# zhixuan-lin/IODINE

Measured on AMD Instinct MI355X. Metric: refinement_iters_per_s, higher is better.
Workload: dtype f32 tensors; conv products from 3 f16 MFMAs on hi+lo splits: >= 22 bits relative to the 8x16-cell maximum (tile-relative), f32 accumulate; 1 GPU; CLEVR6 128x128, K=7, T=5, batch 32/GPU, train step (forward + backward + fused Adam step, noise drawn inside the step); step=train, global_batch=32, slots=7, iters=5, img_size=128, hip_graph=False

## Files before the change

iodine_amd/csrc/iodine_testops.cpp:

```cpp
#include "iodine_internal.h"

namespace {

class OpScratch {
    char* base_ = nullptr;
    std::vector<size_t> off_;
public:
    OpScratch(const char* who, std::initializer_list<size_t> region_bytes)
    {
        size_t total = 0;
        for (size_t b : region_bytes) { off_.push_back(total); total += (b + 15) & ~(size_t)15; }
        const hipError_t e = hipMalloc((void**)&base_, std::max<size_t>(total, 16));
        if (e != hipSuccess) { base_ = nullptr; free_fail(IODINE_ERR_HIP, std::string(who) + ": hipMalloc of " + std::to_string(total) + " bytes of scratch: " + hipGetErrorString(e)); }
    }
    ~OpScratch() { if (base_) (void)hipFree(base_); }
    OpScratch(const OpScratch&) = delete;
    OpScratch& operator=(const OpScratch&) = delete;
    bool ok() const { return base_ != nullptr; }
    template <typename T = float> T* at(int region) const { return reinterpret_cast<T*>(base_ + off_[region]); }
    Pack pack(int region) const { return Pack{at<char>(region), at(region + 1)}; }
};

int op_done(const char* who, hipStream_t st, hipError_t e) { return free_hip(who, e == hipSuccess ? hipStreamSynchronize(st) : e); }

constexpr size_t META_BYTES = 64;

}

extern "C" {

int iodine_op_conv3x3(void* stream, int mode, const float* in, const float* w, const float* bias, const float* aux,
                      float* out, int n, int ih, int iw, int w_o, int w_i, int cin_pad, int cout, int stride, int epi,
                      int tflip)
{
    hipStream_t st = (hipStream_t)stream;
    const bool square_cc = cin_pad == cout && w_o == cout && w_i == cout && ih == iw;
    switch (mode) {
    case IODINE_CONV_S2_FWD: case IODINE_CONV_S2_DGRAD: case IODINE_CONV_S2_FWD_F32: case IODINE_CONV_S2_DGRAD_F32: {
        const bool fwd = mode == IODINE_CONV_S2_FWD || mode == IODINE_CONV_S2_FWD_F32;
        const int f32 = mode == IODINE_CONV_S2_FWD_F32 || mode == IODINE_CONV_S2_DGRAD_F32;
        const int cp = fwd ? (cin_pad == 20 ? 32 : (cin_pad == 12 || cin_pad == 8 ? 16 : cin_pad)) : cin_pad;
        OpScratch scr("iodine_op_conv3x3(s2 f16x3)", {wpk_s2_tile_bytes(cp, cout), META_BYTES});
        if (!scr.ok()) return IODINE_ERR_HIP;
        const Pack p = scr.pack(0);
        hipError_t e = f32 ? launch_pack_conv_weights_s2f32(st, w, w_o, w_i, cp, cout, fwd ? 0 : 2, p.data)
                           : launch_pack_conv_weights_f16(st, w, w_o, w_i, cp, cout, fwd ? 0 : 2, p.meta, p.data);
        if (e == hipSuccess)
            e = fwd ? launch_conv3x3_s2_f16x3(st, in, p.data, p.meta, bias, out, n, ih, cin_pad, cout, nullptr, 0, f32)
                    : launch_conv3x3_s2_dgrad_f16x3(st, in, p.data, p.meta, aux, out, n, ih, cout, f32);
        return op_done("iodine_op_conv3x3(s2 f16x3)", st, e);
    }
    case IODINE_CONV_WS: case IODINE_CONV_WS_B: case IODINE_CONV_WS_1P: {
        if (!square_cc || ih % 16 != 0) return free_fail(IODINE_ERR_INVALID, "iodine_op_conv3x3(ws): shape");
        const size_t tf = conv_ws_tmax_floats(n, ih);
        OpScratch scr("iodine_op_conv3x3(ws)", {wpk_ws_bytes(cout), META_BYTES, tf * sizeof(float), tf * sizeof(float)});
        if (!scr.ok()) return IODINE_ERR_HIP;
        const Pack p = scr.pack(0);
        float *tin = scr.at(2), *tout = scr.at(3);
        hipError_t e = launch_pack_conv_weights_ws(st, w, cout, tflip, p.meta, p.data);
        if (e == hipSuccess) e = launch_cell_max(st, in, tin, n, ih, cout);
        if (e == hipSuccess) e = launch_conv3x3_ws_f16x3(st, in, p.data, p.meta, bias, aux, out, tin, tout, n, ih, cout, epi, 0, mode == IODINE_CONV_WS_1P ? 1 : 3);
        return op_done("iodine_op_conv3x3(ws)", st, e);
    }
    case IODINE_CONV_S2WS: case IODINE_CONV_S2WS_F32: {
        if (!square_cc || !conv3x3_s2ws_ok(ih, cout)) return free_fail(IODINE_ERR_INVALID, "iodine_op_conv3x3(s2ws): shape");
        const bool f32 = mode == IODINE_CONV_S2WS_F32;
        OpScratch scr("iodine_op_conv3x3(s2ws)", {wpk_ws_bytes(cout), META_BYTES});
        if (!scr.ok()) return IODINE_ERR_HIP;
        const Pack p = scr.pack(0);
        hipError_t e = f32 ? launch_pack_conv_weights_ws32(st, w, cout, 0, p.data) : launch_pack_conv_weights_ws(st, w, cout, 0, p.meta, p.data);
        if (e == hipSuccess) e = launch_conv3x3_s2ws_f16x3(st, in, p.data, p.meta, bias, out, n, ih, cout, f32);
        return op_done("iodine_op_conv3x3(s2ws)", st, e);
    }
    case IODINE_CONV_WS_F32: {
        if (!square_cc || ih % 16 != 0) return free_fail(IODINE_ERR_INVALID, "iodine_op_conv3x3(ws f32): shape");
        OpScratch scr("iodine_op_conv3x3(ws f32)", {wpk_ws_bytes(cout)});
        if (!scr.ok()) return IODINE_ERR_HIP;
        hipError_t e = launch_pack_conv_weights_ws32(st, w, cout, tflip, scr.at<char>(0));
        if (e == hipSuccess) e = launch_conv3x3_ws_f32(st, in, scr.at<char>(0), bias, aux, out, n, ih, cout, epi, 0);
        return op_done("iodine_op_conv3x3(ws f32)", st, e);
    }
#ifdef IODINE_WITH_WINO
    case IODINE_CONV_WINO: {
        if (!square_cc || ih % 16 != 0) return free_fail(IODINE_ERR_INVALID, "iodine_op_conv3x3(wino): shape");
        const size_t tf = conv_ws_tmax_floats(n, ih);
        OpScratch scr("iodine_op_conv3x3(wino)", {conv_wino_wpk_bytes(cout), META_BYTES, tf * sizeof(float), tf * sizeof(float), conv_wino_scratch_floats(cout) * sizeof(float)});
        if (!scr.ok()) return IODINE_ERR_HIP;
        const Pack p = scr.pack(0);
        float *tin = scr.at(2), *tout = scr.at(3);
        hipError_t e = launch_pack_conv_weights_wino(st, w, cout, tflip, p.meta, p.data, scr.at(4));
        if (e == hipSuccess) e = launch_cell_max(st, in, tin, n, ih, cout);
        if (e == hipSuccess) e = launch_conv3x3_wino_f16x3(st, in, p.data, p.meta, bias, aux, out, tin, tout, n, ih, cout, epi, 0);
        return op_done("iodine_op_conv3x3(wino)", st, e);
    }
#endif
    case IODINE_CONV_TILE_F16: {
        OpScratch scr("iodine_op_conv3x3(f16x3)", {wpk_tile_f16_bytes(cin_pad, cout), META_BYTES});
        if (!scr.ok()) return IODINE_ERR_HIP;
        const Pack p = scr.pack(0);
        hipError_t e = launch_pack_conv_weights_f16(st, w, w_o, w_i, cin_pad, cout, tflip, p.meta, p.data);
        if (e == hipSuccess) e = launch_conv3x3_tile_f16x3(st, in, p.data, p.meta, bias, aux, out, n, ih, cin_pad, cout, epi, 0);
        return op_done("iodine_op_conv3x3(f16x3)", st, e);
    }
    default: break;
    }
    OpScratch scr("iodine_op_conv3x3", {wpk_tile_f32_bytes(cin_pad, cout)});
    if (!scr.ok()) return IODINE_ERR_HIP;
    float* wpk = scr.at(0);
    hipError_t e = launch_pack_conv_weights(st, w, w_o, w_i, cin_pad, cout, tflip, wpk);
    if (e == hipSuccess && mode == IODINE_CONV_TILE_F32)
        e = (ih == iw && stride == 1) ? launch_conv3x3_tile(st, in, wpk, bias, aux, out, n, ih, cin_pad, cout, epi) : hipErrorInvalidValue;
    else if (e == hipSuccess)
        e = launch_conv3x3_gather(st, in, wpk, bias, out, n, ih, iw, cin_pad, cout, stride);
    return op_done("iodine_op_conv3x3", st, e);
}

int iodine_op_dec_out(void* stream, const float* in, const float* w, const float* bias, float* out, int n, int s, int c)
{
    hipStream_t st = (hipStream_t)stream;
    OpScratch scr("iodine_op_dec_out", {wpk_out_taps_bytes(c)});
    if (!scr.ok()) return IODINE_ERR_HIP;
    hipError_t e = launch_pack_dec_out(st, w, scr.at(0), c);
    if (e == hipSuccess) e = launch_dec_out(st, in, scr.at(0), bias, out, n, s, c);
    return op_done("iodine_op_dec_out", st, e);
}

int iodine_op_dec_out_f16x3(void* stream, const float* in, const float* w, const float* bias, float* out, int n, int s, int c, int variant)
{
    hipStream_t st = (hipStream_t)stream;
    if (s % 16 != 0 || (c != 64 && c != 32)) return free_fail(IODINE_ERR_INVALID, "iodine_op_dec_out_f16x3: shape");
    OpScratch scr("iodine_op_dec_out_f16x3", {std::max(wpk_out_gemm_bytes(c), wpk_out_rows32_bytes(c)), META_BYTES, conv_ws_tmax_floats(n, s) * sizeof(float)});
    if (!scr.ok()) return IODINE_ERR_HIP;
    const Pack p = scr.pack(0);
    float* tin = scr.at(2);
    hipError_t e = launch_pack_dec_out_gemm(st, w, c, p.meta, p.data);
    if (e == hipSuccess) e = launch_cell_max(st, in, tin, n, s, c);
    if (e == hipSuccess && variant == IODINE_DEC_OUT_ROWS_F32) {
        e = launch_pack_dec_out_rows32(st, w, c, (float*)p.data);
        if (e == hipSuccess) e = launch_dec_out_rows_f16x3(st, in, p.data, nullptr, bias, out, n, s, c, nullptr, 1);
    } else if (e == hipSuccess)
        e = variant == IODINE_DEC_OUT_ROWS ? launch_dec_out_rows_f16x3(st, in, p.data, p.meta, bias, out, n, s, c, tin)
                                           : launch_dec_out_stream_f16x3(st, in, p.data, p.meta, bias, out, n, s, c, variant == IODINE_DEC_OUT_TILES_NOMAX ? nullptr : tin);
    return op_done("iodine_op_dec_out_f16x3", st, e);
}

int iodine_op_conv3x3_wgrad(void* stream, const float* in, const float* d, float* gw, float* gb, int n, int s, int ci_pad,
                            int ci_real, int co, int stride)
{
    hipStream_t st = (hipStream_t)stream;
    const int cmax = std::max(std::max(ci_pad, co), 32);
    OpScratch scr("iodine_op_conv3x3_wgrad", {sizeof(float) * 512 * 4 * 9 * cmax * cmax, sizeof(float) * WGRAD_FOLD * 9 * cmax * cmax, sizeof(float) * 512 * 64});
    if (!scr.ok()) return IODINE_ERR_HIP;
    float *part = scr.at(0), *fold = scr.at(1), *part_b = scr.at(2);
    int nparts = 0, cip = 0, nb = 0;
    hipError_t e;
    if (stride == 1 && co == 4) {
        e = launch_dec_out_wgrad_gemm_f16x3(st, in, d, part, part_b, n, s, ci_pad, &nparts, &nb);
        if (e == hipSuccess) e = launch_wgrad_reduce(st, part, nparts, ci_pad, 4, 4, ci_real, ci_real, 1.f, gw, fold);
    } else if (stride == 1) {
        e = launch_conv3x3_wgrad_f16x3_ws(st, in, d, part, part_b, n, s, ci_pad, co, &nparts, &cip, &nb);
        if (e == hipSuccess) e = launch_wgrad_reduce(st, part, nparts, ci_pad, cip, co, ci_real, ci_real, 1.f, gw, fold);
    } else {
        e = launch_conv3x3_s2_wgrad_f16x3(st, in, d, part, part_b, n, s, ci_pad, co, &nparts, &cip, &nb, nullptr, 0, stride == IODINE_WGRAD_STRIDE2_F32);
        if (e == hipSuccess) e = launch_wgrad_reduce(st, part, nparts, cip, co, co, ci_real, ci_real, 1.f, gw, fold);
    }
    if (e == hipSuccess) e = launch_colsum(st, part_b, nb, co, co, 1.f, gb);
    return op_done("iodine_op_conv3x3_wgrad", st, e);
}

int iodine_op_gen_conv(void* stream, int mode, const float* in, const float* w, const float* bias, const float* aux, float* out, float* gb,
                       int n, int si, int ci, int ldc, int co, int k, int s, int elu)
{
    hipStream_t st = (hipStream_t)stream;
    if (mode < IODINE_GEN_FWD || mode > IODINE_GEN_WGRAD || s < 1 || s > 8 || (k != 3 && k != 5 && k != 7) || ldc < ci) return free_fail(IODINE_ERR_INVALID, "iodine_op_gen_conv: argument");
    const unsigned chmask = (elu & 0x100) ? ((unsigned)elu >> 9) : 0xffffffffu;
    elu &= 1;
    OpScratch scr("iodine_op_gen_conv", {wpk_gen_bytes(k, ldc, co), mode == IODINE_GEN_WGRAD ? gen_wgrad_scratch_floats(ci, co, k) * sizeof(float) : 0});
    if (!scr.ok()) return IODINE_ERR_HIP;
    float* wt = scr.at(0);
    hipError_t e = hipSuccess;
    if (mode == IODINE_GEN_FWD) {
        e = launch_gen_pack_weights(st, w, co, ci, k, wt);
        if (e == hipSuccess) e = launch_gen_conv_fwd(st, in, wt, bias, out, n, si, ci, ldc, co, k, s, elu, chmask);
    } else if (mode == IODINE_GEN_DGRAD) {
        e = launch_gen_pack_weights(st, w, co, ldc, k, wt);
        if (e == hipSuccess) e = launch_gen_conv_dgrad(st, in, wt, aux, out, n, si, ci, ldc, co, k, s);
    } else {
        e = launch_gen_conv_wgrad(st, in, aux, scr.at(1), n, si, ci, ldc, ci, co, k, s, 1.f, out, gb, chmask);
    }
    return op_done("iodine_op_gen_conv", st, e);
}

int iodine_op_gen_conv_tier(int mode, int si, int ci, int ldc, int co, int k, int s)
{
    if (mode < IODINE_GEN_FWD || mode > IODINE_GEN_WGRAD || si < 1 || ci < 1 || co < 1 || s < 1 || s > 8 || (k != 3 && k != 5 && k != 7) || ldc < ci) return -1;
    const GenTierSel sel = gen_conv_tier(mode, si, ci, ldc, co, k, s);
    return (int)sel.tier | (sel.np << 8) | (sel.seg << 16);
}

int iodine_op_gen_l0(void* stream, int mode, const float* z, const float* w, const float* bias, const float* dpre, float* out, float* gw,
                     float* gb, float* dz, int n, int L, int s, int co, int k, int ld, float alpha)
{
    hipStream_t st = (hipStream_t)stream;
    if (mode < IODINE_GEN_FWD || mode > IODINE_GEN_DGRAD || n < 1 || L < 1 || s < 1 || co < 1 || k < 1 || k > GEN_L0_KMAX || k % 2 == 0 || !z || !w
        || (mode == IODINE_GEN_FWD && (!bias || !out)) || (mode == IODINE_GEN_DGRAD && (!dpre || !dz || ld < L || (alpha != 0.f && (!gw || !gb)))))
        return free_fail(IODINE_ERR_INVALID, "iodine_op_gen_l0: argument");
    OpScratch scr("iodine_op_gen_l0", {wpk_gen_bytes(k, L + 2, co), (size_t)s * sizeof(float), mode == IODINE_GEN_FWD ? (size_t)s * s * co * sizeof(float) : 0,
                                       gen_l0_scratch_floats(n, s, co, k) * sizeof(float)});
    if (!scr.ok()) return IODINE_ERR_HIP;
    float *wt = scr.at(0), *lin = scr.at(1), *cterm = scr.at(2), *tmp = scr.at(3);
    std::vector<float> hlin((size_t)s);
    iodine_linspace_host(s, hlin.data());
    hipError_t e = hipMemcpyAsync(lin, hlin.data(), (size_t)s * sizeof(float), hipMemcpyHostToDevice, st);
    if (e == hipSuccess) e = hipStreamSynchronize(st);
// ... 230 lines not shown
```

iodine_amd/csrc/kernels_convws.hip:

```cpp
#include "common.h"
#include "pack_bodies.h"
#include <cstdio>
#include <vector>

__global__ void pack_conv_weights_ws_kernel(const float* __restrict__ src, int C, int tflip, const float* __restrict__ meta,
                                            _Float16* __restrict__ dst)
{
    const float scale = meta[0];
    const size_t total = pack_ws_total(C);
    for (size_t idx = (size_t)blockIdx.x * blockDim.x + threadIdx.x; idx < total; idx += (size_t)gridDim.x * blockDim.x)
        dst[idx] = pack_ws_element(src, C, tflip, scale, idx);
}

__global__ __launch_bounds__(1024) void weight_scale_ws_kernel(const float* __restrict__ w, int n, float* __restrict__ meta)
{
    __shared__ float s_red[16];
    weight_scale_block(w, n, meta, s_red);
}

hipError_t launch_pack_conv_weights_ws(hipStream_t st, const float* src, int C, int tflip, float* meta, void* dst)
{
    hipLaunchKernelGGL(weight_scale_ws_kernel, dim3(1), dim3(1024), 0, st, src, C * C * 9, meta);
    const size_t total = wpk_ws_vecs(C) * 8;
    hipLaunchKernelGGL(pack_conv_weights_ws_kernel, dim3((unsigned)((total + 255) / 256)), dim3(256), 0, st, src, C, tflip,
                       meta, (_Float16*)dst);
    return hipGetLastError();
}

__global__ __launch_bounds__(256) void cell_max_kernel(const float* __restrict__ x, float* __restrict__ tmax, int S, int C)
{
    const int cells_x = S / 16, cells_y = S / 8;
    const int cell = blockIdx.x;
    const int cx = cell % cells_x, cy = (cell / cells_x) % cells_y, n = cell / (cells_x * cells_y);
    const float4* base = reinterpret_cast<const float4*>(x + (size_t)n * S * S * C);
    const int c4 = C / 4;
    float m = 0.f;
    for (int i = threadIdx.x; i < 128 * c4; i += 256) {
        const int px = i / c4, q = i % c4;
        const float4 v = base[((size_t)(cy * 8 + px / 16) * S + cx * 16 + px % 16) * c4 + q];
        m = fmaxf(m, fmaxf(fmaxf(fabsf(v.x), fabsf(v.y)), fmaxf(fabsf(v.z), fabsf(v.w))));
    }
    __shared__ float s_red[4];
    m = wave_max_f32(m);
    if ((threadIdx.x & 63) == 0) s_red[threadIdx.x >> 6] = m;
    __syncthreads();
    if (threadIdx.x < 4) tmax[(size_t)cell * 4 + threadIdx.x] = fmaxf(fmaxf(s_red[0], s_red[1]), fmaxf(s_red[2], s_red[3]));
}

hipError_t launch_cell_max(hipStream_t st, const float* x, float* tmax, int N, int S, int C)
{
    hipLaunchKernelGGL(cell_max_kernel, dim3(N * (S / 16) * (S / 8)), dim3(256), 0, st, x, tmax, S, C);
    return hipGetLastError();
}

#ifdef IODINE_TILE_PROF
__device__ unsigned g_ws_prof[TP_MAXBLK * 8];
__device__ unsigned long long g_ws_ts[TP_MAXBLK * 16];
__device__ unsigned long long g_ws_se[TP_MAXBLK * 2];
static void ws_prof_dump(hipStream_t st, int blocks, int ntiles);
#endif

template <int SEGS>
IOD_DEVINL float pixel_lane_sum(float v)
{
    {
        const auto r = __builtin_amdgcn_permlane32_swap(__float_as_uint(v), __float_as_uint(v), false, false);
        v = __uint_as_float(r[0]) + __uint_as_float(r[1]);
    }
    {
        const auto r = __builtin_amdgcn_permlane16_swap(__float_as_uint(v), __float_as_uint(v), false, false);
        v = __uint_as_float(r[0]) + __uint_as_float(r[1]);
    }
    if constexpr (SEGS == 8) v += __uint_as_float(__builtin_amdgcn_update_dpp(0u, __float_as_uint(v), 0x128, 0xf, 0xf, false));
    return v;
}

constexpr int ws_pxb(int c) { return 160; }
constexpr int ws_bpc(int c, int epi) { return 2; }

template <int C, int EPI, bool F32 = false, int NPROD = 3>
__global__ __launch_bounds__(256, ws_bpc(C, EPI))
void conv3x3_ws_f16x3_kernel(const float* __restrict__ in, const uint4* __restrict__ wpk, const float* __restrict__ wmeta,
                             const float* __restrict__ bias, const float* __restrict__ aux, float* __restrict__ out,
                             const float* __restrict__ tmax_in, float* __restrict__ tmax_out, int S, int lgS, int ntiles, int rev)
{
    constexpr int NCG = C / 16;
    constexpr int NPG = 4 / NCG;
    constexpr int RW = 8 / NPG;
    constexpr int NCHUNK = C / 32;
    constexpr int HC = 18, HR = 10, NPX = HC * HR;
    constexpr int PXB = ws_pxb(C);
    constexpr int EPS = C * 4 + 32;
    constexpr int BUFB = ((NPX + 1) * PXB > 128 * EPS ? (NPX + 1) * PXB : 128 * EPS);
    constexpr int NIN = (NPX * 8 + 255) / 256;
    constexpr int NS = (RW + 2) * 3;
    constexpr bool XPOSE = true;
    constexpr bool ROWS = EPI == EPI_L0ROWS || EPI == EPI_L0ROWSX;
    constexpr int NQ = EPI == EPI_L0ROWSX ? 4 : 3;
    constexpr bool GRADF = EPI == EPI_MUL_ELUGRAD || ROWS;
    constexpr int SEGS = C / 4, PPI = 64 / SEGS, NEP = 32 / PPI;
    static_assert(C == 64 || C == 32, "channel counts of the shipped decoders");
    static_assert(EPI == EPI_BIAS_ELU || EPI == EPI_MUL_ELUGRAD || ROWS, "epilogue");
    static_assert(NPROD == 3 || (NPROD == 1 && !F32), "products per term: the split (3) or hi.hi alone (1, fp16 form only)");
    constexpr bool ONE = NPROD == 1;

    extern __shared__ __attribute__((aligned(16))) unsigned char smem_b[];

    using std::integral_constant;
    const int tid = threadIdx.x, lane = tid & 63;
    const int wv = __builtin_amdgcn_readfirstlane(tid >> 6);
    const int cg = wv % NCG, pg = wv / NCG;
    const int lpx = lane & 15, lkb = lane >> 4;

#define WS_BLOAD4(dst, voff, rsrc, soff) \
    asm volatile("buffer_load_dwordx4 %0, %1, %2, %3 offen" : "=v"(dst) : "v"(voff), "s"(rsrc), "s"(soff) : "memory")
#ifndef WS_STORE_POLICY
#define WS_STORE_POLICY 0
#endif
#if WS_STORE_POLICY == 1
#define WS_STORE_MOD " nt"
#elif WS_STORE_POLICY == 2
#define WS_STORE_MOD " sc1"
#elif WS_STORE_POLICY == 3
#define WS_STORE_MOD " sc0 sc1"
#else
#define WS_STORE_MOD ""
#endif
#define WS_BSTORE4(src, voff, rsrc, soff) \
    asm volatile("s_nop 4\n\tbuffer_store_dwordx4 %0, %1, %2, %3 offen" WS_STORE_MOD "\n\ts_nop 1" :: "v"(src), "v"(voff), "s"(rsrc), "s"(soff) : "memory")
#define WS_SGPR_SETTLE(rsrc, soff) asm volatile("s_nop 4" :: "s"(rsrc), "s"(soff) : "memory")

    using wreg_t = std::conditional_t<F32, f32x4, f16x8>;
    wreg_t wh[NCHUNK][9], wl[NCHUNK][9];
    auto load_weights = [&]() {
        const uint4* wp = wpk + (size_t)cg * NCHUNK * 9 * 2 * 64 + lane;
#pragma unroll
        for (int c = 0; c < NCHUNK; ++c)
#pragma unroll
            for (int t = 0; t < 9; ++t) {
                if constexpr (ONE) {
                    const uint4 h = wp[((c * 9 + t) * 2 + 0) * 64];
                    __builtin_memcpy(&wh[c][t], &h, 16);
                } else {
                const uint4 h = wp[((c * 9 + t) * 2 + 0) * 64], l = wp[((c * 9 + t) * 2 + 1) * 64];
                __builtin_memcpy(&wh[c][t], &h, 16);
                __builtin_memcpy(&wl[c][t], &l, 16);
                }
            }
#pragma unroll
        for (int c = 0; c < NCHUNK; ++c)
#pragma unroll
            for (int t = 0; t < 9; ++t) {
                if constexpr (ONE) asm volatile("" : "+v"(wh[c][t]));
                else asm volatile("" : "+v"(wh[c][t]), "+v"(wl[c][t]));
            }
    };
    float inv_w = 1.f;
    if constexpr (!F32) inv_w = wmeta[1];
    const float xstep_u = __uint_as_float(__builtin_amdgcn_readfirstlane(__float_as_uint(__fdiv_rn(2.f, (float)(S - 1)))));
    (void)xstep_u;

    const unsigned lds_base = (unsigned)(size_t)(__attribute__((address_space(3))) unsigned char*)smem_b;
    const unsigned lw0 = (unsigned)((tid >> 3) * PXB + (tid & 7) * (F32 ? 16 : 8));
    const bool last_idle = tid + (NIN - 1) * 256 >= NPX * 8;
    const unsigned fr_base = lds_base + (unsigned)(((pg * RW) * HC + lpx) * PXB + lkb * 16);

    const int tiles_x = S >> 4, tiles_y = S >> 3, lg_tx = lgS - 4, lg_tpi = 2 * lgS - 7;
    const int nblk = gridDim.x;
    const int xcd = blockIdx.x & 7, bix = blockIdx.x >> 3, bpx = (nblk + 7) >> 3;
    const int per_xcd = (ntiles + 7) >> 3;
    const int t_begin = xcd * per_xcd, t_end = min(ntiles, t_begin + per_xcd);

    f32x4 rin[NIN];
    auto tile_coords = [&](int t, int& n, int& ty, int& tx) {
        const int tt = rev ? ntiles - 1 - t : t;
        n = tt >> lg_tpi;
        ty = (tt >> lg_tx) & (tiles_y - 1); tx = tt & (tiles_x - 1);
    };
    float tmv = 0.f;
    auto issue_tmax = [&](int t) {
        int n, ty, tx;
        tile_coords(t, n, ty, tx);
        const int cell = min(lane >> 2, 8);
        const int cy = min(max(ty + cell / 3 - 1, 0), tiles_y - 1), cx = min(max(tx + cell % 3 - 1, 0), tiles_x - 1);
        const float* p = tmax_in + ((((size_t)n << lg_tpi) + (cy << lg_tx) + cx) << 2) + (lane & 3);
        asm volatile("global_load_dword %0, %1, off" : "=v"(tmv) : "v"(p) : "memory");
    };
    auto issue_loads = [&](int t, int chunk) {
        int n, ty, tx;
        tile_coords(t, n, ty, tx);
        const i32x4 rsrc = iod_make_rsrc(in + (size_t)n * S * S * C, (unsigned)(S * S * C * 4));
        unsigned goff[NIN];
#pragma unroll
        for (int k = 0; k < NIN; ++k) {
            const int px = (tid >> 3) + 32 * k;
            const int hy = (px * 3641) >> 16, hx = px - hy * HC;
            const int gy = ty * 8 - 1 + hy, gx = tx * 16 - 1 + hx;
            const bool ok = (k < NIN - 1 || px < NPX) && (unsigned)gy < (unsigned)S && (unsigned)gx < (unsigned)S;
            goff[k] = ok ? (unsigned)(((((gy << lgS) + gx) * C) << 2) + ((tid & 7) << 4)) : 0x80000000u;
        }
        const int soff = chunk * 128;
        WS_SGPR_SETTLE(rsrc, soff);
#pragma unroll
        for (int k = 0; k < NIN; ++k) WS_BLOAD4(rin[k], goff[k], rsrc, soff);
    };
    const int t0 = t_begin + bix;
    const int nstage = t0 < t_end ? ((t_end - t0 + bpx - 1) / bpx) * NCHUNK : 0;
    auto issue_stage = [&](int s) {
        const int t = t0 + (s / NCHUNK) * bpx, c = s % NCHUNK;
        issue_loads(t, c);
        if constexpr (!F32) { if (c == 0) issue_tmax(t); }
    };
    auto vm_wait = [&](auto nc) {
        constexpr int nleft = decltype(nc)::value;
        asm volatile("s_waitcnt vmcnt(%0)" :: "n"(nleft) : "memory");
#pragma unroll
        for (int k = 0; k < NIN; ++k) asm volatile("" : "+v"(rin[k]));
        asm volatile("" : "+v"(tmv));
        __builtin_amdgcn_sched_barrier(0);
    };

    f32x4 acc[RW];

    auto convert_k = [&](auto kc, int buf, float scale) {
        constexpr int k = decltype(kc)::value;
        unsigned char* sb = smem_b + buf * BUFB;
        f32x4 v = rin[k];
        if constexpr (F32) {
            const unsigned o32 = (k == NIN - 1 && last_idle) ? (unsigned)(NPX * PXB) : lw0 + (unsigned)(k * 32 * PXB);
            *reinterpret_cast<f32x4*>(sb + o32) = v;
        } else if constexpr (ONE) {
            v.x *= scale; v.y *= scale; v.z *= scale; v.w *= scale;
            typedef _Float16 hr2 __attribute__((ext_vector_type(2)));
            const hr2 h01 = {(_Float16)v.x, (_Float16)v.y}, h23 = {(_Float16)v.z, (_Float16)v.w};
            uint2 hi;
            __builtin_memcpy(&hi.x, &h01, 4); __builtin_memcpy(&hi.y, &h23, 4);
            const unsigned o = (k == NIN - 1 && last_idle) ? (unsigned)(NPX * PXB) : lw0 + (unsigned)(k * 32 * PXB);
            *reinterpret_cast<uint2*>(sb + o) = hi;
        } else {
        v.x *= scale; v.y *= scale; v.z *= scale; v.w *= scale;
        typedef __fp16 h2 __attribute__((ext_vector_type(2)));
        const h2 h01 = __builtin_amdgcn_cvt_pkrtz(v.x, v.y), h23 = __builtin_amdgcn_cvt_pkrtz(v.z, v.w);
        const h2 l01 = __builtin_amdgcn_cvt_pkrtz(v.x - (float)h01.x, v.y - (float)h01.y), l23 = __builtin_amdgcn_cvt_pkrtz(v.z - (float)h23.x, v.w - (float)h23.y);
        uint2 hi, lo;
        __builtin_memcpy(&hi.x, &h01, 4); __builtin_memcpy(&hi.y, &h23, 4);
        __builtin_memcpy(&lo.x, &l01, 4); __builtin_memcpy(&lo.y, &l23, 4);
        const unsigned o = (k == NIN - 1 && last_idle) ? (unsigned)(NPX * PXB) : lw0 + (unsigned)(k * 32 * PXB);
        *reinterpret_cast<uint2*>(sb + o) = hi;
        *reinterpret_cast<uint2*>(sb + o + 64) = lo;
        }
    };

    constexpr int NST = ROWS ? 2 * NQ : NEP + (F32 ? 0 : 1);

#define WS_DSR128(dst, addr, off) asm volatile("ds_read_b128 %0, %1 offset:%2" : "=v"(dst) : "v"(addr), "n"(off))
    struct Frag { wreg_t h, l; };
    constexpr int HOOK0 = 3;
    auto compute = [&](auto cc, int buf, bool has_next, bool next_after_epi, float next_scale_same, float& next_scale, bool has_next2,
                       int next2_stage) {
        constexpr int c = decltype(cc)::value;
        const unsigned base = fr_base + (unsigned)(buf * BUFB);
        Frag f[2];
        auto LOADF = [](auto sc, Frag& fr, unsigned b) {
            constexpr int s = decltype(sc)::value;
            constexpr int hr = s / 3, dx = s % 3;
            constexpr int off = (hr * HC + dx) * PXB;
            WS_DSR128(fr.h, b, off);
            if constexpr (!ONE) WS_DSR128(fr.l, b, off + 64);
        };
        auto MMA = [&](auto sc, const Frag& fr) {
            constexpr int s = decltype(sc)::value;
            constexpr int hr = s / 3, dx = s % 3;
            if constexpr (F32) {
#pragma unroll
                for (int j = 0; j < 4; ++j)
#pragma unroll
                    for (int dy = 0; dy < 3; ++dy) {
                        const int y = hr - dy;
                        if (y >= 0 && y < RW) acc[y] = __builtin_amdgcn_mfma_f32_16x16x4f32(wh[c][dy * 3 + dx][j], fr.h[j], acc[y], 0, 0, 0);
                    }
#pragma unroll
                for (int j = 0; j < 4; ++j)
#pragma unroll
                    for (int dy = 0; dy < 3; ++dy) {
                        const int y = hr - dy;
                        if (y >= 0 && y < RW) acc[y] = __builtin_amdgcn_mfma_f32_16x16x4f32(wl[c][dy * 3 + dx][j], fr.l[j], acc[y], 0, 0, 0);
                    }
            } else if constexpr (ONE) {
#pragma unroll
                for (int dy = 0; dy < 3; ++dy) {
                    const int y = hr - dy;
                    if (y >= 0 && y < RW) acc[y] = __builtin_amdgcn_mfma_f32_16x16x32_f16(wh[c][dy * 3 + dx], fr.h, acc[y], 0, 0, 0);
                }
            } else {
#pragma unroll
            for (int dy = 0; dy < 3; ++dy) {
                const int y = hr - dy;
                if (y >= 0 && y < RW) acc[y] = __builtin_amdgcn_mfma_f32_16x16x32_f16(wh[c][dy * 3 + dx], fr.l, acc[y], 0, 0, 0);
            }
#pragma unroll
            for (int dy = 0; dy < 3; ++dy) {
                const int y = hr - dy;
                if (y >= 0 && y < RW) acc[y] = __builtin_amdgcn_mfma_f32_16x16x32_f16(wl[c][dy * 3 + dx], fr.h, acc[y], 0, 0, 0);
            }
#pragma unroll
            for (int dy = 0; dy < 3; ++dy) {
                const int y = hr - dy;
                if (y >= 0 && y < RW) acc[y] = __builtin_amdgcn_mfma_f32_16x16x32_f16(wh[c][dy * 3 + dx], fr.h, acc[y], 0, 0, 0);
            }
            }
        };
        LOADF(integral_constant<int, 0>{}, f[0], base);
        auto step = [&](auto sc) {
            constexpr int s = decltype(sc)::value;
            if constexpr (s + 1 < NS) {
                LOADF(integral_constant<int, (s + 1 < NS ? s + 1 : 0)>{}, f[(s + 1) & 1], base);
                if constexpr (ONE) asm volatile("s_waitcnt lgkmcnt(1)" ::: "memory");
                else asm volatile("s_waitcnt lgkmcnt(2)" ::: "memory");
            } else {
                asm volatile("s_waitcnt lgkmcnt(0)" ::: "memory");
            }
            if constexpr (ONE) asm volatile("" : "+v"(f[s & 1].h));
            else asm volatile("" : "+v"(f[s & 1].h), "+v"(f[s & 1].l));
            __builtin_amdgcn_sched_barrier(0);
#ifndef WS_ABL_NOMFMA
            MMA(sc, f[s & 1]);
#endif
            if constexpr (s == HOOK0) {
                if (has_next) {
                    if (next_after_epi) vm_wait(integral_constant<int, NST>{});
                    else vm_wait(integral_constant<int, 0>{});
                    if constexpr (!F32) next_scale = c + 1 < NCHUNK ? next_scale_same : fresh_scale(wave_max_f32(lane < 36 ? tmv : 0.f));
                }
            }
            if constexpr (s > HOOK0 && s <= HOOK0 + NIN) {
                if (has_next) convert_k(integral_constant<int, s - HOOK0 - 1>{}, buf ^ 1, next_scale);
            }
            if constexpr (s == HOOK0 + NIN + 1) {
                if (has_next2) issue_stage(next2_stage);
            }
            __builtin_amdgcn_sched_barrier(0);
        };
        static_for<NS>(step);
    };
#undef WS_DSR128

    if (nstage == 0) return;
#ifdef IODINE_TILE_PROF
    if (tid == 0 && blockIdx.x < TP_MAXBLK) g_ws_se[blockIdx.x * 2] = __builtin_amdgcn_s_memtime();
#endif
#ifdef WS_ROLEPRIO
    {
        unsigned hwid;
        asm volatile("s_getreg_b32 %0, hwreg(HW_REG_HW_ID)" : "=s"(hwid));
        if (hwid & 1u) __builtin_amdgcn_s_setprio(WS_ROLEPRIO);
    }
#endif
#ifndef WS_ALTPRIO
#define WS_ALTPRIO 2
#endif
#ifndef WS_ALT_SH32
#define WS_ALT_SH32 18
#endif
#ifndef WS_ALT_SH16
#define WS_ALT_SH16 16
#endif
#if !defined(WS_ALTTIME) && !defined(WS_ALTTILES)
#define WS_ALTTIME 1
#endif
#if WS_ALTPRIO > 0
    unsigned role;
    { unsigned hwid; asm volatile("s_getreg_b32 %0, hwreg(HW_REG_HW_ID)" : "=s"(hwid)); role = hwid & 1u; }
#endif
    TP_DECL;
    issue_stage(0);
    load_weights();
    vm_wait(integral_constant<int, 0>{});
    float cur_scale = 1.f;
    if constexpr (!F32) cur_scale = fresh_scale(wave_max_f32(lane < 36 ? tmv : 0.f));
    static_for<NIN>([&](auto kc) { convert_k(kc, 0, cur_scale); });
    if (nstage > 1) issue_stage(1);
    bool first = true;
    float next_scale = cur_scale;
#ifdef WS_PRIO
    __builtin_amdgcn_s_setprio(WS_PRIO);
#endif
    for (int s0 = 0; s0 < nstage; s0 += NCHUNK) {
#if WS_ALTPRIO > 0
#ifdef WS_ALTTIME
        if ((((unsigned)(__builtin_amdgcn_s_memtime() >> (F32 ? WS_ALT_SH32 : WS_ALT_SH16))) ^ role) & 1u) __builtin_amdgcn_s_setprio(2); else __builtin_amdgcn_s_setprio(0);
#else
        if ((((unsigned)(s0 / NCHUNK) / WS_ALTPRIO) ^ role) & 1u) __builtin_amdgcn_s_setprio(2); else __builtin_amdgcn_s_setprio(0);
#endif
#endif
        const int t = t0 + (s0 / NCHUNK) * bpx;
        int n, ty, tx;
        tile_coords(t, n, ty, tx);
#pragma unroll
        for (int y = 0; y < RW; ++y) acc[y] = f32x4{0.f, 0.f, 0.f, 0.f};
        TP_STAMP(0);
#ifdef IODINE_TILE_PROF
        { const int ti = s0 / NCHUNK - 20; if (tid == 0 && ti >= 0 && ti < 8 && blockIdx.x < TP_MAXBLK) g_ws_ts[blockIdx.x * 16 + 2 * ti] = __builtin_amdgcn_s_memtime(); }
#endif
#pragma unroll
        for (int c = 0; c < NCHUNK; ++c) {
            const int s = s0 + c;
            __syncthreads();
            TP_STAMP(1);
#ifdef WS_PRIO
            __builtin_amdgcn_s_setprio(0);
#endif
            const bool after_epi = c == 0 && !first;
            if (c == 0) compute(integral_constant<int, 0>{}, s & 1, s + 1 < nstage, after_epi, cur_scale, next_scale, s + 2 < nstage, s + 2);
            else compute(integral_constant<int, (NCHUNK > 1 ? 1 : 0)>{}, s & 1, s + 1 < nstage, after_epi, cur_scale, next_scale, s + 2 < nstage, s + 2);
#ifdef WS_PRIO
            __builtin_amdgcn_s_setprio(WS_PRIO);
#endif
            TP_STAMP(2);
        }
        first = false;
#ifdef IODINE_TILE_PROF
        { const int ti = s0 / NCHUNK - 20; if (tid == 0 && ti >= 0 && ti < 8 && blockIdx.x < TP_MAXBLK) g_ws_ts[blockIdx.x * 16 + 2 * ti + 1] = __builtin_amdgcn_s_memtime(); }
#endif
        const float inv = inv_w / cur_scale;
        cur_scale = next_scale;
        const i32x4 rsrc_out = iod_make_rsrc(out + (size_t)n * S * S * C, (unsigned)(S * S * C * 4));
        if constexpr (XPOSE) {
            unsigned char* sb = smem_b + ((s0 + NCHUNK - 1) & 1) * BUFB;
            const int seg = lane % SEGS, pl = lane / SEGS;
            const unsigned vbase = (unsigned)(((((ty * 8 + 2 * wv) << lgS) + tx * 16 + pl) * C + seg * 4) * 4);
            f32x4 ax[GRADF ? NEP : 1];
            if constexpr (GRADF) {
                const i32x4 rsrc_aux = iod_make_rsrc(aux + (size_t)n * S * S * C, (unsigned)(S * S * C * 4));
#pragma unroll
                for (int j = 0; j < NEP / 2; ++j) {
                    const int soff = ((((j * PPI) / 16) << lgS) + (j * PPI) % 16) * C * 4;
                    WS_SGPR_SETTLE(rsrc_aux, soff);
                    WS_BLOAD4(ax[j], vbase, rsrc_aux, soff);
                }
            }
            __syncthreads();
            TP_STAMP(3);
#pragma unroll
            for (int y = 0; y < RW; ++y)
                *reinterpret_cast<f32x4*>(sb + ((pg * RW + y) * 16 + lpx) * EPS + (16 * cg + 4 * lkb) * 4) = acc[y] * inv;
            if constexpr (GRADF) {
                const i32x4 rsrc_aux = iod_make_rsrc(aux + (size_t)n * S * S * C, (unsigned)(S * S * C * 4));
#pragma unroll
                for (int j = NEP / 2; j < NEP; ++j) {
                    const int soff = ((((j * PPI) / 16) << lgS) + (j * PPI) % 16) * C * 4;
                    WS_SGPR_SETTLE(rsrc_aux, soff);
                    WS_BLOAD4(ax[j], vbase, rsrc_aux, soff);
                }
            }
            f32x4 b4 = f32x4{0.f, 0.f, 0.f, 0.f};
            if constexpr (EPI == EPI_BIAS_ELU) {
                const float4 tb = *reinterpret_cast<const float4*>(bias + seg * 4);
                b4 = f32x4{tb.x, tb.y, tb.z, tb.w};
            }
            __syncthreads();
            TP_STAMP(4);
            float vmax = 0.f;
            const unsigned char* sr = sb + ((2 * wv) * 16 + pl) * EPS + seg * 16;
            constexpr int PB = GRADF ? NEP / 2 : NEP;
            constexpr int XJ0 = EPI == EPI_L0ROWSX ? NEP / 2 : NEP;
            f32x4 rxw = f32x4{0.f, 0.f, 0.f, 0.f};
            (void)rxw;
            auto lin_at = [&](int x) {
                return x < (S >> 1) ? __fadd_rn(-1.f, __fmul_rn(xstep_u, (float)x)) : __fsub_rn(1.f, __fmul_rn(xstep_u, (float)(S - 1 - x)));
            };
            auto xw_row_done = [&](int row) {
#pragma unroll
                for (int e = 0; e < 4; ++e) rxw[e] = pixel_lane_sum<SEGS>(rxw[e]);
                if (pl == 0) {
                    float* rpx = out + ((((size_t)n * S + ty * 8 + 2 * wv + row) * tiles_x + tx) * NQ) * C + seg * 4;
                    *reinterpret_cast<f32x4*>(rpx + 3 * C) = rxw;
                }
            };
            (void)lin_at; (void)xw_row_done;
            f32x4 pv[PB];
            f32x4 rtot = f32x4{0.f, 0.f, 0.f, 0.f};
            (void)rtot;
            static_for<NEP>([&](auto jc) {
                constexpr int j = decltype(jc)::value;
                if constexpr (j % PB == 0) {
#pragma unroll
                    for (int i = 0; i < PB; ++i) pv[i] = *reinterpret_cast<const f32x4*>(sr + (j + i) * PPI * EPS);
                }
                f32x4 v = pv[j % PB];
                if constexpr (EPI == EPI_BIAS_ELU) {
                    v = f32x4{elu1_fast(v.x + b4.x), elu1_fast(v.y + b4.y), elu1_fast(v.z + b4.z), elu1_fast(v.w + b4.w)};
                } else {
                    f32x4& axj = ax[j];
                    constexpr int IPRW = 16 / PPI;
                    asm volatile("s_waitcnt vmcnt(%0)" :: "n"(ROWS ? NEP - 1 - j + 3 * (j / IPRW) + (j % IPRW ? 1 : 0) : NEP - 1) : "memory");
                    asm volatile("" : "+v"(axj));
                    v.x *= elu1_grad_from_out(axj.x); v.y *= elu1_grad_from_out(axj.y);
                    v.z *= elu1_grad_from_out(axj.z); v.w *= elu1_grad_from_out(axj.w);
                }
                if constexpr (EPI == EPI_L0ROWSX) {
                    constexpr int IPRX = 16 / PPI;
                    if constexpr (j < XJ0) {
#ifndef WS_ABL_X_NOWB
                        *reinterpret_cast<f32x4*>(const_cast<unsigned char*>(sr) + j * PPI * EPS) = v;
#endif
                    } else {
#ifndef WS_ABL_X_NOINLINE
                        const float xwj = lin_at(tx * 16 + pl + (j % IPRX) * PPI);
                        if constexpr (j % IPRX == 0) rxw = v * xwj;
                        else rxw += v * xwj;
                        if constexpr (j % IPRX == IPRX - 1) xw_row_done(j / IPRX);
#endif
                    }
                }
                if constexpr (ROWS) {
                    constexpr int IPR = 16 / PPI;
                    const bool lt = tx == 0, rt = tx == tiles_x - 1;
                    const f32x4 zero = f32x4{0.f, 0.f, 0.f, 0.f};
                    float* rp = out + ((((size_t)n * S + ty * 8 + 2 * wv + j / IPR) * tiles_x + tx) * NQ) * C + seg * 4;
                    if constexpr (j % IPR == 0) {
                        const bool isl = lt && pl == 0;
                        if (pl == 0) *reinterpret_cast<f32x4*>(rp) = isl ? v : zero;
                        rtot = isl ? zero : v;
                    } else if constexpr (j % IPR == IPR - 1) {
                        const bool isr = rt && pl == PPI - 1;
                        f32x4 Rb = isr ? v : zero, tot = rtot + (isr ? zero : v);
#pragma unroll
                        for (int e = 0; e < 4; ++e) tot[e] = pixel_lane_sum<SEGS>(tot[e]);
                        if (rt) {
#pragma unroll
                            for (int e = 0; e < 4; ++e) Rb[e] = pixel_lane_sum<SEGS>(Rb[e]);
                        }
                        if (pl == 0) {
                            *reinterpret_cast<f32x4*>(rp + C) = tot;
                            *reinterpret_cast<f32x4*>(rp + 2 * C) = Rb;
                        }
                    } else {
                        rtot += v;
                    }
                } else {
                    vmax = fmaxf(vmax, fmaxf(fmaxf(fabsf(v.x), fabsf(v.y)), fmaxf(fabsf(v.z), fabsf(v.w))));
                    const unsigned vb = vbase; const i32x4 ro = rsrc_out;
                    const int soff = ((((j * PPI) / 16) << lgS) + (j * PPI) % 16) * C * 4;
#ifdef WS_ABL_NOSTORE
                    asm volatile("" :: "v"(v), "v"(vb), "s"(ro), "s"(soff) : "memory");
#else
                    WS_BSTORE4(v, vb, ro, soff);
#endif
                }
            });
#ifndef WS_ABL_X_NOPASSB
            if constexpr (EPI == EPI_L0ROWSX) {
                constexpr int IPRX = 16 / PPI;
                static_assert(XJ0 == IPRX && XJ0 <= PB, "one tile row, one LDS read batch");
#pragma unroll
                for (int i = 0; i < XJ0; ++i) pv[i] = *reinterpret_cast<const f32x4*>(sr + i * PPI * EPS);
#pragma unroll
                for (int i = 0; i < XJ0; ++i) {
                    const float xwj = lin_at(tx * 16 + pl + i * PPI);
                    if (i == 0) rxw = pv[i] * xwj;
                    else rxw += pv[i] * xwj;
                }
                xw_row_done(0);
            }
#endif
            if constexpr (!ROWS && !F32) {
                vmax = wave_max_f32(vmax);
                const int tt = rev ? ntiles - 1 - t : t;
                float* tp = tmax_out + (size_t)tt * 4 + wv;
                asm volatile("global_store_dword %0, %1, off\n\ts_nop 1" :: "v"(tp), "v"(vmax) : "memory");
            }
            TP_STAMP(5);
        }
    }
    TP_FLUSH(g_ws_prof);
#ifdef IODINE_TILE_PROF
    if (tid == 0 && blockIdx.x < TP_MAXBLK) {
        unsigned hwid, xcc;
        asm volatile("s_getreg_b32 %0, hwreg(HW_REG_HW_ID)" : "=s"(hwid));
        asm volatile("s_getreg_b32 %0, hwreg(HW_REG_XCC_ID)" : "=s"(xcc));
        g_ws_prof[blockIdx.x * 8 + 6] = hwid; g_ws_prof[blockIdx.x * 8 + 7] = xcc;
        g_ws_se[blockIdx.x * 2 + 1] = __builtin_amdgcn_s_memtime();
    }
#endif
#undef WS_BLOAD4
#undef WS_BSTORE4
#undef WS_SGPR_SETTLE
}

template <int C, int EPI, bool F32 = false, int NPROD = 3>
static hipError_t launch_ws_inst(hipStream_t st, const float* in, const void* wpk, const float* wmeta, const float* bias,
                                 const float* aux, float* out, const float* tmax_in, float* tmax_out, int N, int S, int rev)
{
    constexpr size_t buf_in = (size_t)(18 * 10 + 1) * ws_pxb(C), buf_out = (size_t)128 * (C * 4 + 32);
    constexpr size_t lds = 2 * (buf_in > buf_out ? buf_in : buf_out);
    int n_cu = 0;
    if (hipError_t e = iod_cu_count(&n_cu); e != hipSuccess) return e;
    int lgS = 0;
    while ((1 << lgS) < S) ++lgS;
    const int ntiles = N * (S / 16) * (S / 8);
    int bpc = ws_bpc(C, EPI);
#ifdef WS_TUNE_ENV
    if (const char* e = getenv("IODINE_WS_BPC")) bpc = atoi(e);
#endif
    const int blocks = iod_xcd_grid(ntiles, bpc, n_cu);
    const hipError_t e = iod_launch<conv3x3_ws_f16x3_kernel<C, EPI, F32, NPROD>>(st, dim3(blocks), dim3(256), lds, (int)lds, in,
                                                                                 reinterpret_cast<const uint4*>(wpk), wmeta, bias, aux, out, tmax_in,
                                                                                 tmax_out, S, lgS, ntiles, rev);
#ifdef IODINE_TILE_PROF
    ws_prof_dump(st, blocks, ntiles);
#endif
    return e;
}

#ifdef IODINE_TILE_PROF
static void ws_prof_dump(hipStream_t st, int blocks, int ntiles)
{
    static const char* names[8] = {"bookkeeping", "stage-barrier", "taps+staging-hooks", "epi-barrier", "tile->lds+barrier", "epilogue", "-", "-"};
    const std::vector<unsigned> hp = tp_report(st, HIP_SYMBOL(g_ws_prof), blocks,
                                               tp_title("[ws prof] memtime ticks per block (wave 0, %d tiles)", (ntiles + blocks - 1) / blocks).c_str(), names, 8);
    const int nb = (int)(hp.size() / 8);
    if (getenv("IODINE_WS_TS")) {
        std::vector<unsigned long long> ts((size_t)nb * 16);
        (void)hipMemcpyFromSymbol(ts.data(), HIP_SYMBOL(g_ws_ts), ts.size() * sizeof(unsigned long long));
        for (int b2 = 0; b2 < 4 && b2 + 256 < nb; ++b2) {
            const unsigned long long base = ts[(size_t)b2 * 16];
            fprintf(stderr, "blk %d   :", b2);
            for (int i = 0; i < 16; ++i) fprintf(stderr, " %lld", (long long)(ts[(size_t)b2 * 16 + i] - base));
            fprintf(stderr, "\nblk %d :", b2 + 256);
            for (int i = 0; i < 16; ++i) fprintf(stderr, " %lld", (long long)(ts[(size_t)(b2 + 256) * 16 + i] - base));
            fprintf(stderr, "\n");
        }
    }
    if (getenv("IODINE_WS_SE")) {
        std::vector<unsigned long long> se((size_t)nb * 2);
        (void)hipMemcpyFromSymbol(se.data(), HIP_SYMBOL(g_ws_se), se.size() * sizeof(unsigned long long));
        unsigned long long t0 = ~0ull;
        for (int b2 = 0; b2 < nb; ++b2) t0 = std::min(t0, se[(size_t)b2 * 2]);
        std::vector<long long> st_(nb), en_(nb);
        for (int b2 = 0; b2 < nb; ++b2) { st_[b2] = (long long)(se[(size_t)b2 * 2] - t0); en_[b2] = (long long)(se[(size_t)b2 * 2 + 1] - t0); }
        std::vector<long long> es(en_), ss(st_);
        std::sort(es.begin(), es.end()); std::sort(ss.begin(), ss.end());
        fprintf(stderr, "[ws prof] block start: median %lld max %lld | block end: min %lld p25 %lld median %lld p75 %lld max %lld\n", ss[nb / 2], ss[nb - 1],
                es[0], es[nb / 4], es[nb / 2], es[3 * nb / 4], es[nb - 1]);
        int shown = 0;
        for (int a = 0; a < nb && shown < 6; ++a)
            for (int c2 = a + 1; c2 < nb; ++c2) {
                const unsigned ha = hp[(size_t)a * 8 + 6], hc = hp[(size_t)c2 * 8 + 6];
                if ((hp[(size_t)a * 8 + 7] & 0xf) == (hp[(size_t)c2 * 8 + 7] & 0xf) && ((ha >> 8) & 0xff) == ((hc >> 8) & 0xff)) {
                    fprintf(stderr, "  CU pair blocks %d / %d: start %lld / %lld end %lld / %lld (wave slots %u / %u)\n", a, c2, st_[a], st_[c2], en_[a], en_[c2],
                            ha & 0xf, hc & 0xf);
                    ++shown;
                    break;
                }
            }
    }
    if (getenv("IODINE_WS_HWID")) {
        for (int b2 = 0; b2 < nb; ++b2) {
            const unsigned hw = hp[(size_t)b2 * 8 + 6], xc = hp[(size_t)b2 * 8 + 7];
            fprintf(stderr, "blk %d xcc %u se %u sh %u cu %u simd %u wave %u\n", b2, xc & 0xf, (hw >> 13) & 7, (hw >> 12) & 1, (hw >> 8) & 0xf,
                    (hw >> 4) & 3, hw & 0xf);
        }
    }
}
#endif

hipError_t launch_conv3x3_ws_f16x3(hipStream_t st, const float* in, const void* wpk, const float* wmeta, const float* bias,
                                   const float* aux, float* out, const float* tmax_in, float* tmax_out, int N, int S, int c,
                                   int epi, int rev, int products)
{
    if (S < 16 || (S & (S - 1)) != 0 || !tmax_in || (epi != EPI_L0ROWS && epi != EPI_L0ROWSX && !tmax_out)) return hipErrorInvalidValue;
    if (products != 1 && products != 3) return hipErrorInvalidValue;
    return iod_dispatch<64, 32>(c, [&](auto cc) {
        return iod_dispatch<EPI_BIAS_ELU, EPI_MUL_ELUGRAD, EPI_L0ROWS, EPI_L0ROWSX>(epi, [&](auto ep) {
            return iod_dispatch<3, 1>(products, [&](auto np) {
                return launch_ws_inst<cc, ep, false, np>(st, in, wpk, wmeta, bias, aux, out, tmax_in, tmax_out, N, S, rev);
            });
        });
    });
}

__global__ void pack_conv_weights_ws32_kernel(const float* __restrict__ src, int C, int tflip, float* __restrict__ dst)
{
    const size_t total = wpk_ws_vecs(C) * 4;
    const int nchunk = C / 32;
    for (size_t idx = (size_t)blockIdx.x * blockDim.x + threadIdx.x; idx < total; idx += (size_t)gridDim.x * blockDim.x) {
        const int j = idx & 3;
        size_t r = idx >> 2;
        const int lane = r & 63; r >>= 6;
        const int hl = r & 1; r >>= 1;
        const int tap = r % 9; r /= 9;
        const int c = r % nchunk;
        const int cg = (int)(r / nchunk);
        const int co = 16 * cg + (lane & 15), ci = 32 * c + 16 * hl + 4 * (lane >> 4) + j;
        dst[idx] = tflip ? src[((size_t)ci * C + co) * 9 + (8 - tap)] : src[((size_t)co * C + ci) * 9 + tap];
    }
}

hipError_t launch_pack_conv_weights_ws32(hipStream_t st, const float* src, int C, int tflip, void* dst)
{
    const size_t total = wpk_ws_vecs(C) * 4;
    hipLaunchKernelGGL(pack_conv_weights_ws32_kernel, dim3((unsigned)((total + 255) / 256)), dim3(256), 0, st, src, C, tflip, (float*)dst);
    return hipGetLastError();
}

hipError_t launch_conv3x3_ws_f32(hipStream_t st, const float* in, const void* wpk, const float* bias, const float* aux, float* out,
                                 int N, int S, int c, int epi, int rev)
{
    if (S < 16 || (S & (S - 1)) != 0) return hipErrorInvalidValue;
    return iod_dispatch<64, 32>(c, [&](auto cc) {
        return iod_dispatch<EPI_BIAS_ELU, EPI_MUL_ELUGRAD, EPI_L0ROWS, EPI_L0ROWSX>(epi, [&](auto ep) {
            return launch_ws_inst<cc, ep, true>(st, in, wpk, nullptr, bias, aux, out, nullptr, nullptr, N, S, rev);
        });
    });
}
```

Before: 3352 image-refinement-iters/s.

## Park one weight fragment in LDS across the epilogue for the L0ROWSX conv

For the C=64 L0ROWSX three-product weight-stationary conv, one hi/lo weight fragment is spilled to a dedicated LDS region after loading and reloaded at the end of each tile epilogue. This frees VGPRs during the epilogue. The epilogue now accumulates the x-weighted row sums inline for every row instead of writing half of them back to LDS and doing a second pass, and it folds the ELU-grad multiply into an FMA for the row total. It also switches the tmax load to a scalar-base addressed form and passes rev for the plain WS test op. In exchange LDS per block grows, and every tile adds LDS traffic plus a wait on the fragment reload.

Result: no change. 3356 image-refinement-iters/s, median of 6 (+0.1%).

```diff
diff --git a/iodine_amd/csrc/iodine_testops.cpp b/iodine_amd/csrc/iodine_testops.cpp
--- a/iodine_amd/csrc/iodine_testops.cpp
+++ b/iodine_amd/csrc/iodine_testops.cpp
@@ -59,7 +59,8 @@
         float *tin = scr.at(2), *tout = scr.at(3);
         hipError_t e = launch_pack_conv_weights_ws(st, w, cout, tflip, p.meta, p.data);
         if (e == hipSuccess) e = launch_cell_max(st, in, tin, n, ih, cout);
-        if (e == hipSuccess) e = launch_conv3x3_ws_f16x3(st, in, p.data, p.meta, bias, aux, out, tin, tout, n, ih, cout, epi, 0, mode == IODINE_CONV_WS_1P ? 1 : 3);
+        const int rev = mode == IODINE_CONV_WS;
+        if (e == hipSuccess) e = launch_conv3x3_ws_f16x3(st, in, p.data, p.meta, bias, aux, out, tin, tout, n, ih, cout, epi, rev, mode == IODINE_CONV_WS_1P ? 1 : 3);
         return op_done("iodine_op_conv3x3(ws)", st, e);
     }
     case IODINE_CONV_S2WS: case IODINE_CONV_S2WS_F32: {
diff --git a/iodine_amd/csrc/kernels_convws.hip b/iodine_amd/csrc/kernels_convws.hip
--- a/iodine_amd/csrc/kernels_convws.hip
+++ b/iodine_amd/csrc/kernels_convws.hip
@@ -77,6 +77,7 @@
 
 constexpr int ws_pxb(int c) { return 160; }
 constexpr int ws_bpc(int c, int epi) { return 2; }
+constexpr int ws_park_bytes(int c, int epi, int nprod) { return epi == EPI_L0ROWSX && c == 64 && nprod != 1 ? 256 * 16 : 0; }
 
 template <int C, int EPI, bool F32 = false, int NPROD = 3>
 __global__ __launch_bounds__(256, ws_bpc(C, EPI))
@@ -103,6 +104,10 @@
     static_assert(EPI == EPI_BIAS_ELU || EPI == EPI_MUL_ELUGRAD || ROWS, "epilogue");
     static_assert(NPROD == 3 || (NPROD == 1 && !F32), "products per term: the split (3) or hi.hi alone (1, fp16 form only)");
     constexpr bool ONE = NPROD == 1;
+    constexpr bool PARK = ws_park_bytes(C, EPI, NPROD) != 0;
+    constexpr int PARK_C = NCHUNK - 1, PARK_T = 0;
+    constexpr int PARK0 = (NPX + 1) * PXB, PARK1 = 2 * BUFB;
+    static_assert(!PARK || (NCHUNK == 2 && PARK0 % 16 == 0 && PARK0 + 256 * 16 <= BUFB && PARK1 - PARK0 < 65536), "parked fragments");
 
     extern __shared__ __attribute__((aligned(16))) unsigned char smem_b[];
 
@@ -183,6 +188,11 @@
         tile_coords(t, n, ty, tx);
         const int cell = min(lane >> 2, 8);
         const int cy = min(max(ty + cell / 3 - 1, 0), tiles_y - 1), cx = min(max(tx + cell % 3 - 1, 0), tiles_x - 1);
+        if constexpr (PARK) {
+            const unsigned po = (unsigned)((((n << lg_tpi) + (cy << lg_tx) + cx) << 2) + (lane & 3)) << 2;
+            asm volatile("s_nop 4\n\tglobal_load_dword %0, %1, %2" : "=v"(tmv) : "v"(po), "s"(tmax_in) : "memory");
+            return;
+        }
         const float* p = tmax_in + ((((size_t)n << lg_tpi) + (cy << lg_tx) + cx) << 2) + (lane & 3);
         asm volatile("global_load_dword %0, %1, off" : "=v"(tmv) : "v"(p) : "memory");
     };
@@ -310,6 +320,9 @@
             }
             }
         };
+        if constexpr (PARK && c == PARK_C) {
+            asm volatile("s_waitcnt lgkmcnt(0)" : "+v"(wl[PARK_C][PARK_T]), "+v"(wh[PARK_C][PARK_T]) :: "memory");
+        }
         LOADF(integral_constant<int, 0>{}, f[0], base);
         auto step = [&](auto sc) {
             constexpr int s = decltype(sc)::value;
@@ -376,6 +389,12 @@
     issue_stage(0);
     load_weights();
     vm_wait(integral_constant<int, 0>{});
+    const unsigned park_addr = lds_base + (unsigned)PARK0 + (unsigned)tid * 16u;
+    (void)park_addr;
+    if constexpr (PARK) {
+        *reinterpret_cast<wreg_t*>(smem_b + PARK0 + tid * 16) = wh[PARK_C][PARK_T];
+        *reinterpret_cast<wreg_t*>(smem_b + PARK1 + tid * 16) = wl[PARK_C][PARK_T];
+    }
     float cur_scale = 1.f;
     if constexpr (!F32) cur_scale = fresh_scale(wave_max_f32(lane < 36 ? tmv : 0.f));
     static_for<NIN>([&](auto kc) { convert_k(kc, 0, cur_scale); });
@@ -463,7 +482,6 @@
             float vmax = 0.f;
             const unsigned char* sr = sb + ((2 * wv) * 16 + pl) * EPS + seg * 16;
             constexpr int PB = GRADF ? NEP / 2 : NEP;
-            constexpr int XJ0 = EPI == EPI_L0ROWSX ? NEP / 2 : NEP;
             f32x4 rxw = f32x4{0.f, 0.f, 0.f, 0.f};
             (void)rxw;
             auto lin_at = [&](int x) {
@@ -481,6 +499,8 @@
             f32x4 pv[PB];
             f32x4 rtot = f32x4{0.f, 0.f, 0.f, 0.f};
             (void)rtot;
+            f32x4 vraw = f32x4{0.f, 0.f, 0.f, 0.f}, vfac = vraw;
+            (void)vraw; (void)vfac;
             static_for<NEP>([&](auto jc) {
                 constexpr int j = decltype(jc)::value;
                 if constexpr (j % PB == 0) {
@@ -493,25 +513,23 @@
                 } else {
                     f32x4& axj = ax[j];
                     constexpr int IPRW = 16 / PPI;
-                    asm volatile("s_waitcnt vmcnt(%0)" :: "n"(ROWS ? NEP - 1 - j + 3 * (j / IPRW) + (j % IPRW ? 1 : 0) : NEP - 1) : "memory");
+                    asm volatile("s_waitcnt vmcnt(%0)" :: "n"(ROWS ? NEP - 1 - j + NQ * (j / IPRW) + (j % IPRW ? 1 : 0) : NEP - 1) : "memory");
                     asm volatile("" : "+v"(axj));
+                    if constexpr (EPI == EPI_L0ROWSX) {
+                        vraw = v;
+                        vfac = f32x4{elu1_grad_from_out(axj.x), elu1_grad_from_out(axj.y), elu1_grad_from_out(axj.z), elu1_grad_from_out(axj.w)};
+                        v.x *= vfac.x; v.y *= vfac.y; v.z *= vfac.z; v.w *= vfac.w;
+                    } else {
                     v.x *= elu1_grad_from_out(axj.x); v.y *= elu1_grad_from_out(axj.y);
                     v.z *= elu1_grad_from_out(axj.z); v.w *= elu1_grad_from_out(axj.w);
+                    }
                 }
                 if constexpr (EPI == EPI_L0ROWSX) {
                     constexpr int IPRX = 16 / PPI;
-                    if constexpr (j < XJ0) {
-#ifndef WS_ABL_X_NOWB
-                        *reinterpret_cast<f32x4*>(const_cast<unsigned char*>(sr) + j * PPI * EPS) = v;
-#endif
-                    } else {
-#ifndef WS_ABL_X_NOINLINE
-                        const float xwj = lin_at(tx * 16 + pl + (j % IPRX) * PPI);
-                        if constexpr (j % IPRX == 0) rxw = v * xwj;
-                        else rxw += v * xwj;
-                        if constexpr (j % IPRX == IPRX - 1) xw_row_done(j / IPRX);
-#endif
-                    }
+                    const float xwj = lin_at(tx * 16 + pl + (j % IPRX) * PPI);
+                    if constexpr (j % IPRX == 0) rxw = v * xwj;
+                    else rxw += v * xwj;
+                    if constexpr (j % IPRX == IPRX - 1) xw_row_done(j / IPRX);
                 }
                 if constexpr (ROWS) {
                     constexpr int IPR = 16 / PPI;
@@ -536,10 +554,15 @@
                             *reinterpret_cast<f32x4*>(rp + 2 * C) = Rb;
                         }
                     } else {
-                        rtot += v;
+                        if constexpr (EPI == EPI_L0ROWSX) {
+                            rtot = __builtin_elementwise_fma(vraw, vfac, rtot);
+                            asm volatile("" : "+v"(rtot));
+                        } else {
+                            rtot += v;
+                        }
                     }
                 } else {
-                    vmax = fmaxf(vmax, fmaxf(fmaxf(fabsf(v.x), fabsf(v.y)), fmaxf(fabsf(v.z), fabsf(v.w))));
+                    vmax =fmaxf(vmax, fmaxf(fmaxf(fabsf(v.x), fabsf(v.y)), fmaxf(fabsf(v.z), fabsf(v.w))));
                     const unsigned vb = vbase; const i32x4 ro = rsrc_out;
                     const int soff = ((((j * PPI) / 16) << lgS) + (j * PPI) % 16) * C * 4;
 #ifdef WS_ABL_NOSTORE
@@ -549,21 +572,10 @@
 #endif
                 }
             });
-#ifndef WS_ABL_X_NOPASSB
-            if constexpr (EPI == EPI_L0ROWSX) {
-                constexpr int IPRX = 16 / PPI;
-                static_assert(XJ0 == IPRX && XJ0 <= PB, "one tile row, one LDS read batch");
-#pragma unroll
-                for (int i = 0; i < XJ0; ++i) pv[i] = *reinterpret_cast<const f32x4*>(sr + i * PPI * EPS);
-#pragma unroll
-                for (int i = 0; i < XJ0; ++i) {
-                    const float xwj = lin_at(tx * 16 + pl + i * PPI);
-                    if (i == 0) rxw = pv[i] * xwj;
-                    else rxw += pv[i] * xwj;
-                }
-                xw_row_done(0);
-            }
-#endif
+            if constexpr (PARK) {
+                asm volatile("ds_read_b128 %0, %2\n\tds_read_b128 %1, %2 offset:%3" : "=v"(wh[PARK_C][PARK_T]), "=v"(wl[PARK_C][PARK_T])
+                             : "v"(park_addr), "n"(PARK1 - PARK0) : "memory");
+            }
             if constexpr (!ROWS && !F32) {
                 vmax = wave_max_f32(vmax);
                 const int tt = rev ? ntiles - 1 - t : t;
@@ -593,7 +605,8 @@
                                  const float* aux, float* out, const float* tmax_in, float* tmax_out, int N, int S, int rev)
 {
     constexpr size_t buf_in = (size_t)(18 * 10 + 1) * ws_pxb(C), buf_out = (size_t)128 * (C * 4 + 32);
-    constexpr size_t lds = 2 * (buf_in > buf_out ? buf_in : buf_out);
+    constexpr size_t lds = 2 * (buf_in > buf_out ? buf_in : buf_out) + ws_park_bytes(C, EPI, NPROD);
+    static_assert(ws_bpc(C, EPI) * lds <= 160 * 1024, "persistent blocks per CU x LDS per block");
     int n_cu = 0;
     if (hipError_t e = iod_cu_count(&n_cu); e != hipSuccess) return e;
     int lgS = 0;
```
